# SmoothKen/knn-svc

Measured on AMD Instinct MI355X. Metric: audio-sec converted/sec (xRT) end-to-end, cold target pool, higher is better.
Workload: dtype f32; 1 GPU; north-star point per rank: 30 s source vs 10 min target pool (20 x 30 s), ckpt_type=mix, post_opt_0.2, cold (pool encoded inside the step); seeded random weights of WavLM-Large (6 layers executed) and the 22.9 M-param generator; nq=1500, np_per_rank=30000, wavlm_batch_chunks=32, pipeline_depth=2

## Files before the change

knn_svc_amd/csrc/conv_gemm.hip:

```cpp
#include "gemm_core.h"
#include "gemm3_core.h"
#include "gemm2_core.h"

namespace {

thread_local const char* g_last_epilogue = "";
thread_local const char* g_last_kernel = "";

struct ConvArgs {
    const float* x; long x_bstride, x_gstride; int ldx, t_in, cin, taps, stride, dil, pad; float a_slope;
    const float* w; long w_gstride; int n;
    const float* bias; long bias_gstride; int bias_period;
    float* out; long o_bstride, o_gstride; int ldo, m;
    int act; float act_slope;
    const float* resid; long r_bstride, r_gstride; int ldr;
    int accumulate; float div;
    int groups;
    int convt_u, convt_cout, convt_pad, t_out;
    int K;
    const unsigned short* w3;
    const unsigned short* w2;
    int x_split;
    int out_split;
    int split_from;
// ... 693 lines not shown
#pragma unroll
        for (int it = 0; it < TRIPS; ++it) {
            f32x4 v = *(const lds_f4*)(patch + (it * RSTEP + row_in_trip) * PITCH + c) + bias4;
            if (RES) v += rv[it];
            const int m = mrow0 + it * RSTEP;
            bool ok = nv;
            int off;
            if (CONVT) {
                const int o = m * a.convt_u + phase - a.convt_pad;
                ok = ok && m < a.m && o >= 0 && o < a.t_out;
                off = (o * a.ldo + col) * 4;
            } else off = (m * a.ldo + n) * 4;
            if (a.out_absmax && (!CONVT || ok)) {
#pragma unroll
                for (int e = 0; e < 4; ++e) { const unsigned ab = abs_bits(v[e]); amax = ab > amax ? ab : amax; }
            }
            __builtin_amdgcn_raw_buffer_store_b128(__builtin_bit_cast(u32x4, v), o_rsrc, ok ? off : OOB, 0, 0);
        }
    }
    if (a.out_absmax) publish_absmax(a.out_absmax, amax);
}

template <class G>
__device__ __forceinline__ void conv_gemm2win_body(ConvArgs& a, float* lds) {
    resolve_scales(a);
    const int z = blockIdx.z;
    const int nbz = (int)gridDim.z / a.groups;
    const int g = z / nbz, b = z - g * nbz;
    int m0, n0;
    if (!patch_order_decode<G::BM, G::BN>(a.plain, a.m, a.n, m0, n0)) return;
    const float* xz = a.x + b * a.x_bstride + g * a.x_gstride;
    const unsigned short* wz = a.w2 + (long)g * a.n * (a.K / 32) * 64;

    typename G::acc_t acc[G::TM][G::TN];
    KN_ZERO_ACC(acc, G::TM, G::TN, G::NR)
    Split2BLoader<G::B_P, G::B_PIECES> bl(a.n, a.K, n0, threadIdx.x);
    const int tid = threadIdx.x;
    const int w_off0 = ((m0 - a.pad + (tid >> 3)) * a.ldx + (tid & 7) * 4) * 4;
    if constexpr (G::DEEP)
        G::mainloop_deep(lds, a.cin / 32, a.taps, a.dil, w_off0, a.ldx * 4, bl, acc, FastALoader<1>::desc(a, xz),
                         Split2BLoader<G::B_P, G::B_PIECES>::desc(wz, a.n, a.K), a.a_scale, a.a_slope);
    else
        G::mainloop(lds, a.cin / 32, a.taps, a.dil, w_off0, a.ldx * 4, bl, acc, FastALoader<1>::desc(a, xz),
                    Split2BLoader<G::B_P, G::B_PIECES>::desc(wz, a.n, a.K), a.a_scale, a.a_slope);
    if (a.wide) {
        __syncthreads();
        if (a.resid) conv_epilogue_wide32<G, true>(a, acc, lds, m0, n0, b, g);
        else conv_epilogue_wide32<G, false>(a, acc, lds, m0, n0, b, g);
    } else conv_epilogue_any<G>(a, acc, m0, n0, b, g);
}

template <class G, int MINB>
__global__ __launch_bounds__(256, MINB) void conv_gemm2win_kernel(ConvArgs a) {
    extern __shared__ __attribute__((aligned(16))) float lds[];
    conv_gemm2win_body<G>(a, lds);
}

constexpr int KN_MAX_MULTI = 4;
struct ConvArgsN { ConvArgs b[KN_MAX_MULTI]; };
template <class G, int MINB>
__global__ __launch_bounds__(256, MINB) void conv_gemm2win_multi_kernel(ConvArgsN args) {
    extern __shared__ __attribute__((aligned(16))) float lds[];
    ConvArgs a = args.b[blockIdx.y];
    conv_gemm2win_body<G>(a, lds);
}

template <class G, int MINB>
int launch2win(const ConvArgs* args, int count, int batches, hipStream_t st) {
    const ConvArgs& a = args[0];
    const long gx = cdiv64(a.m, G::BM), gy = cdiv64(a.n, G::BN);
    ConvArgsN ap;
    for (int i = 0; i < KN_MAX_MULTI; ++i) { ap.b[i] = args[i < count ? i : 0]; ap.b[i].plain = patch_order_plain(gx, gy); }
    dim3 grid((unsigned)patch_order_ids(gx, gy), (unsigned)count, (unsigned)(batches * a.groups));
    if (count == 1) {
        if (const int rc = kn_lds_optin<conv_gemm2win_kernel<G, MINB>>(G::LDS_BYTES, "conv_gemm")) return rc;
        hipLaunchKernelGGL((conv_gemm2win_kernel<G, MINB>), grid, dim3(256), G::LDS_BYTES, st, ap.b[0]);
        return knnsvc_check_launch("conv_gemm2win");
    }
    if (const int rc = kn_lds_optin<conv_gemm2win_multi_kernel<G, MINB>>(G::LDS_BYTES, "conv_gemm_multi")) return rc;
    hipLaunchKernelGGL((conv_gemm2win_multi_kernel<G, MINB>), grid, dim3(256), G::LDS_BYTES, st, ap);
    return knnsvc_check_launch("conv_gemm2win_multi");
}

template <class G, int EPI = 0>
__global__ __launch_bounds__(256, 1) void conv_gemm2quad_kernel(ConvArgs a) {
    extern __shared__ __attribute__((aligned(16))) float lds[];
#ifdef KN_QUAD_PROF
    if (threadIdx.x == 0 && blockIdx.x < 8192) kn_quad_prof_buf[blockIdx.x * 4 + 0] = (long long)__builtin_amdgcn_s_memrealtime();
#endif
    resolve_scales(a);
    const int z = blockIdx.z;
    const int b = z / a.groups, g = z - b * a.groups;
    int mt, nt;
    if (!quad_order_decode((int)blockIdx.x, (a.m + G::BM - 1) / G::BM, (a.n + G::BN - 1) / G::BN, mt, nt, (int)blockIdx.z)) return;
    const int m0 = mt * G::BM, n0 = nt * G::BN;
    const float* xz = a.x + b * a.x_bstride + g * a.x_gstride;
    const unsigned short* wz = a.w2 + (long)g * a.n * (a.K / 32) * 64;

    typename G::acc_t acc[G::TM][G::TN];
    KN_ZERO_ACC(acc, G::TM, G::TN, G::NR)
    const int M = a.m, row_step = a.stride * a.ldx * 4, row_pad = a.pad * a.ldx * 4;
    auto row_off = [&](int m) -> int { return m < M ? m * row_step - row_pad : G::OOB_OFF; };
    int c_in_tap = 0, uoff = 0;
    const int cin = a.cin, step_tap = (a.dil * a.ldx - a.cin) * 4;
    auto step = [&](int kt) -> int {
        if (kt > 0) { c_in_tap += 32; uoff += 128; if (c_in_tap == cin) { c_in_tap = 0; uoff += step_tap; } }
        return uoff;
    };
    G::mainloop(lds, a.K / 32, row_off, step, FastALoader<1>::desc(a, xz), uniform_rsrc(wz, (int)((long)a.n * (a.K / 32) * 128)),
                a.n, a.K, m0, n0, acc);
#ifdef KN_T_NOEPI
    { float sink = 0.f;
#pragma unroll
      for (int i = 0; i < G::TM; ++i)
#pragma unroll
          for (int j = 0; j < G::TN; ++j)
#pragma unroll
              for (int r = 0; r < G::NR; ++r) sink += acc[i][j][r];
      if (sink == 123456.789f) a.out[threadIdx.x] = sink; }
#else
    __syncthreads();
#ifdef KN_QUAD_PROF
    if (threadIdx.x == 0 && blockIdx.x < 8192) kn_quad_prof_buf[blockIdx.x * 4 + 2] = (long long)__builtin_amdgcn_s_memrealtime();
#endif
    if constexpr (EPI == 1) conv_epilogue_wide_fast<G, 0, false>(a, acc, lds, m0, n0, b, g);
    else if constexpr (EPI == 2) conv_epilogue_wide_fast<G, 1, false>(a, acc, lds, m0, n0, b, g);
    else if constexpr (EPI == 3) conv_epilogue_wide_fast<G, 0, true>(a, acc, lds, m0, n0, b, g);
    else conv_epilogue_wide<G>(a, acc, lds, m0, n0, b, g);
#ifdef KN_QUAD_PROF
    __builtin_amdgcn_s_waitcnt(0);
    __syncthreads();
    if (threadIdx.x == 0 && blockIdx.x < 8192) kn_quad_prof_buf[blockIdx.x * 4 + 3] = (long long)__builtin_amdgcn_s_memrealtime();
#endif
#endif
}

template <class G, int EPI = 0>
int launch2quad(const ConvArgs& a, int batches, hipStream_t st) {
    if (const int rc = kn_lds_optin<conv_gemm2quad_kernel<G, EPI>>(G::LDS_BYTES, "conv_gemm")) return rc;
    dim3 grid((unsigned)quad_order_ids(cdiv64(a.m, G::BM), cdiv64(a.n, G::BN)), 1, (unsigned)(batches * a.groups));
    hipLaunchKernelGGL((conv_gemm2quad_kernel<G, EPI>), grid, dim3(256), G::LDS_BYTES, st, a);
    return knnsvc_check_launch("conv_gemm2quad");
}

template <class G, bool A2>
int launch2v(const ConvArgs& a, int batches, hipStream_t st) {
    if (const int rc = kn_lds_optin<conv_gemm2_kernel<G, A2>>(G::LDS_BYTES, "conv_gemm")) return rc;
    const long gx = cdiv64(a.m, G::BM), gy = cdiv64(a.n, G::BN);
    ConvArgs ap = a;
    ap.plain = patch_order_plain(gx, gy);
    dim3 grid((unsigned)patch_order_ids(gx, gy), 1, (unsigned)(batches * a.groups));
    hipLaunchKernelGGL((conv_gemm2_kernel<G, A2>), grid, dim3(256), G::LDS_BYTES, st, ap);
    return knnsvc_check_launch("conv_gemm2");
}
template <class G>
int launch2(const ConvArgs& a, int batches, hipStream_t st) {
    return a.x_split ? launch2v<G, true>(a, batches, st) : launch2v<G, false>(a, batches, st);
}

__global__ void split_weight2_kernel(const float* __restrict__ w, long n, int K, float scale, const float* __restrict__ absmax,
                                     unsigned short* __restrict__ out) {
    const long i = (long)blockIdx.x * blockDim.x + threadIdx.x;
    const long groups_per_row = K / 4;
    if (absmax) scale = kn_pick_scale(kn_slot_max(absmax));
    if (i >= n * groups_per_row) return;
    const long row = i / groups_per_row; const int k = (int)(i - row * groups_per_row) * 4;
    g2_u32x2 hi, lo;
    f16x2_split4(*(const f32x4*)(w + row * K + k), scale, hi, lo);
    unsigned short* o = out + row * (long)(K / 32) * 64 + (k / 32) * 64 + (k % 32);
    *(g2_u32x2*)o = hi;
    *(g2_u32x2*)(o + 32) = lo;
}

template <class G>
int launch3(const ConvArgs& a, int batches, hipStream_t st) {
    if (const int rc = kn_lds_optin<conv_gemm3_kernel<G>>(G::LDS_BYTES, "conv_gemm")) return rc;
    dim3 grid((unsigned)cdiv64(a.m, G::BM), (unsigned)cdiv64(a.n, G::BN), (unsigned)(batches * a.groups));
    hipLaunchKernelGGL((conv_gemm3_kernel<G>), grid, dim3(256), G::LDS_BYTES, st, a);
    return knnsvc_check_launch("conv_gemm3");
}

__global__ void split_weight_kernel(const float* __restrict__ w, long n, int K, unsigned short* __restrict__ out) {
    const long i = (long)blockIdx.x * blockDim.x + threadIdx.x;
    const long groups_per_row = K / 4;
    if (i >= n * groups_per_row) return;
    const long row = i / groups_per_row; const int k = (int)(i - row * groups_per_row) * 4;
    const f32x4 v = *(const f32x4*)(w + row * K + k);
    unsigned short* o = out + row * (long)(K / 32) * 96 + (k / 32) * 96 + (k % 32);
#pragma unroll
    for (int e = 0; e < 4; ++e) {
        const unsigned x = __float_as_uint(v[e]);
        const float r1 = v[e] - __uint_as_float(x & 0xFFFF0000u);
        const unsigned y = __float_as_uint(r1);
        const float r2 = r1 - __uint_as_float(y & 0xFFFF0000u);
        o[e] = (unsigned short)(x >> 16);
        o[32 + e] = (unsigned short)(y >> 16);
        o[64 + e] = (unsigned short)(__float_as_uint(r2) >> 16);
    }
}

template <class G, int VEC>
int launch(const ConvArgs& a, int batches, hipStream_t st) {
    dim3 grid((unsigned)cdiv64(a.m, G::BM), (unsigned)cdiv64(a.n, G::BN), (unsigned)(batches * a.groups));
    hipLaunchKernelGGL((conv_gemm_kernel<G, VEC>), grid, dim3(256), G::LDS_BYTES, st, a);
    return knnsvc_check_launch("conv_gemm");
}

using G128 = GemmTile<128, 128, 2, 2, 2, 2>;
using G64 = GemmTile<128, 64, 4, 1, 1, 2>;
using G32 = GemmTile<128, 32, 4, 1, 1, 1>;
using H128 = Gemm3Tile<128, 128, 2, 2, 2, 2>;
using H64 = Gemm3Tile<256, 64, 4, 1, 2, 2>;
using H32 = Gemm3Tile<256, 32, 4, 1, 2, 1>;
using F128 = Gemm2Tile<128, 128, 2, 2, 2, 2>;
using F64S = Gemm2Tile<64, 64, 2, 2, 1, 1>;
using F64 = Gemm2Tile<256, 64, 4, 1, 2, 2>;
using F32 = Gemm2Tile<256, 32, 4, 1, 2, 1>;
using Q256S = Gemm2QuadS;
using W128 = Gemm2Win<128, 128, 2, 2, 2, 2, 64>;
using W160 = Gemm2Win<160, 128, 1, 4, 5, 1, 64>;
using W128S = Gemm2Win<64, 128, 2, 2, 1, 2, 64>;
using W128D = Gemm2Win<64, 128, 2, 2, 1, 2, 64, 1>;
using W64 = Gemm2Win<256, 64, 4, 1, 2, 2, 64>;
using W32 = Gemm2Win<256, 32, 4, 1, 2, 1, 64>;
using W64P = Gemm2Win<256, 64, 4, 1, 2, 2, 128>;

template <class G>
int prepare() {
    int rc = kn_lds_optin<conv_gemm_kernel<G, 8>>(G::LDS_BYTES, "conv_gemm");
    if (!rc) rc = kn_lds_optin<conv_gemm_kernel<G, 4>>(G::LDS_BYTES, "conv_gemm");
    if (!rc) rc = kn_lds_optin<conv_gemm_kernel<G, 1>>(G::LDS_BYTES, "conv_gemm");
    return rc;
}

struct Knobs {
    int quad = 1;
    bool quad_epi = true;
    bool generic_epilogue = false;
    bool win = true;
    bool win_wide = true;
    bool win_small = true, win_deep = true, win160 = true;
    bool gemm_small = true;
    bool loaded = false;
};
Knobs g_knobs;
bool env_off(const char* name) { const char* e = getenv(name); return e && e[0] == '0'; }
void load_knobs() {
    Knobs k;
    const char* q = getenv("KNNSVC_QUAD");
    k.quad = q ? atoi(q) : 1;
    k.quad_epi = !env_off("KNNSVC_QUAD_EPI");
    const char* ep = getenv("KNNSVC_EPILOGUE");
    k.generic_epilogue = ep && ep[0] == 'g';
    k.win = !env_off("KNNSVC_WIN"); k.win_small = !env_off("KNNSVC_WIN_SMALL"); k.win_deep = !env_off("KNNSVC_WIN_DEEP");
    k.win_wide = !env_off("KNNSVC_WIN_WIDE");
    k.win160 = !env_off("KNNSVC_WIN160"); k.gemm_small = !env_off("KNNSVC_GEMM_SMALL");
    k.loaded = true;
    g_knobs = k;
}
const Knobs& knobs() { if (!g_knobs.loaded) load_knobs(); return g_knobs; }

}

extern "C" int knnsvc_reload_knobs(void) { load_knobs(); return KNNSVC_OK; }

static int conv_prep(const knnsvc_conv_desc* d, ConvArgs& a, bool& fast, bool& vec4, bool& quad_ok) {
    KN_REQUIRE(d && d->x && d->w && d->out, "conv_gemm: null operand");
    KN_REQUIRE(d->cin > 0 && d->taps > 0 && d->n > 0 && d->m >= 0 && d->t_in >= 0, "conv_gemm: bad sizes");
    KN_REQUIRE(d->batches > 0 && d->groups > 0, "conv_gemm: batches/groups must be positive");
    KN_REQUIRE((d->ldx >= d->cin || (d->taps == 1 && d->ldx > 0)) && d->stride > 0, "conv_gemm: ldx < cin or stride <= 0");
    KN_REQUIRE((long)d->batches * d->groups <= 65535, "conv_gemm: batches*groups > 65535");
    KN_REQUIRE(cdiv64(d->n, 32) <= 65535, "conv_gemm: n too large for grid.y");
    if (d->convt_u) {
        KN_REQUIRE(d->convt_cout > 0 && d->n % d->convt_cout == 0 && d->n / d->convt_cout == d->convt_u,
                   "conv_gemm: transposed mode needs n == u*cout");
        KN_REQUIRE(d->ldo >= d->convt_cout, "conv_gemm: ldo < cout");
    } else {
        KN_REQUIRE(d->ldo >= d->n, "conv_gemm: ldo < n");
    }
    if (d->resid) KN_REQUIRE(d->ldr > 0, "conv_gemm: resid without ldr");

    a.x = d->x; a.x_bstride = d->x_bstride; a.x_gstride = d->x_gstride; a.ldx = d->ldx; a.t_in = d->t_in;
    a.cin = d->cin; a.taps = d->taps; a.stride = d->stride; a.dil = d->dil; a.pad = d->pad; a.a_slope = d->a_slope;
    a.w = d->w; a.w_gstride = d->w_gstride; a.n = d->n;
    a.bias = d->bias; a.bias_gstride = d->bias_gstride; a.bias_period = d->bias_period;
    a.out = d->out; a.o_bstride = d->o_bstride; a.o_gstride = d->o_gstride; a.ldo = d->ldo; a.m = d->m;
    a.act = d->act; a.act_slope = d->act_slope;
    a.resid = d->resid; a.r_bstride = d->r_bstride; a.r_gstride = d->r_gstride; a.ldr = d->ldr;
    a.accumulate = d->accumulate; a.div = d->div == 0.f ? 1.0f : d->div;
    a.groups = d->groups;
    a.convt_u = d->convt_u; a.convt_cout = d->convt_cout; a.convt_pad = d->convt_pad; a.t_out = d->t_out;
    a.K = d->cin * d->taps;
    a.w3 = (const unsigned short*)d->w_bf16x3;
    a.w2 = (const unsigned short*)d->w_f16x2;
    a.out_scale = 1.0f; a.a_scale = 1.0f; a.w_scale = 1.0f;
    a.x_absmax = nullptr; a.w_absmax = nullptr; a.out_absmax = d->out_absmax; a.x_bound_mul = 1.0f; a.x_bound_add = 0.f;
    a.n_dyn = d->n_dyn; a.dyn_tin_mul = d->dyn_t_in_mul; a.dyn_tin_add = d->dyn_t_in_add; a.dyn_m_mul = d->dyn_m_mul;
    a.dyn_m_add = d->dyn_m_add; a.dyn_tout_mul = d->dyn_t_out_mul;
    if (d->n_dyn) KN_REQUIRE(d->dyn_t_in_mul >= 0 && d->dyn_m_mul >= 0 && d->dyn_t_in_add >= 0 && d->dyn_m_add >= 0 && d->batches == 1,
                             "conv_gemm: dynamic length needs non-negative affine coefficients and batches == 1");
    a.split_scale = d->out_f16x2_scale > 0.f ? d->out_f16x2_scale : KN_F16X2_A_SCALE;
    a.x_split = d->x_f16x2; a.out_split = d->out_f16x2 != 0; a.split_from = d->out_f16x2 > 1 ? d->out_f16x2 : 0;
    KN_REQUIRE(d->out_f16x2 >= 0 && (d->out_f16x2 <= 1 || d->out_f16x2 % 32 == 0), "conv_gemm: out_f16x2 is 0, 1 or the first split column (a multiple of 32)");
    a.wide = 0; a.plain = 0;
    a.lin = !d->convt_u && (long)d->m * d->ldo * 4 < (1L << 31) && (!d->resid || (long)d->m * d->ldr * 4 < (1L << 31)) &&
            !knobs().generic_epilogue;

    vec4 = (d->cin % 4 == 0) && (d->ldx % 4 == 0) && (((uintptr_t)d->x & 15) == 0) &&
                      (((uintptr_t)d->w & 15) == 0) && (d->x_bstride % 4 == 0) && (d->x_gstride % 4 == 0) &&
                      (d->w_gstride % 4 == 0);
    if (const int rc = prepare<G128>()) return rc;
    if (const int rc = prepare<G64>()) return rc;
    if (const int rc = prepare<G32>()) return rc;
    fast = vec4 && (d->cin % 32 == 0) && ((long)d->t_in * d->ldx * 4 < (1L << 30)) &&
                      ((long)d->n * a.K * 4 < (1L << 30)) && ((long)d->m * d->stride * d->ldx * 4 < (1L << 30));
    if (a.out_split)
        KN_REQUIRE(!d->resid && !d->accumulate && a.div == 1.0f && !d->convt_u && d->n % 32 == 0 && d->ldo % 32 == 0 &&
                   ((uintptr_t)d->out & 15) == 0, "conv_gemm: out_f16x2 needs a plain [m, n % 32 == 0] output (no resid/accumulate/div/convt)");
    if (a.out_split) {
        int e2 = 0;
        KN_REQUIRE(frexpf(a.split_scale, &e2) == 0.5f, "conv_gemm: out_f16x2_scale must be a power of two");
        KN_REQUIRE(!a.out_absmax, "conv_gemm: out_absmax is for fp32 outputs (a split output's scale is chosen by the caller)");
    }
    if (a.x_split)
        KN_REQUIRE(fast && a.w2 && d->a_slope == 1.0f,
                   "conv_gemm: x_f16x2 needs the f16x2 fast path (cin % 32 == 0, split weights) and a_slope 1");
    if (fast && a.w2) {
        KN_REQUIRE(d->w_f16x2_scale > 0.f || d->w_absmax, "conv_gemm: w_f16x2 without its scale");
        a.a_scale = d->a_f16x2_scale > 0.f ? d->a_f16x2_scale : KN_F16X2_A_SCALE;
        a.w_scale = d->w_f16x2_scale > 0.f ? d->w_f16x2_scale : 1.0f;
        { int e2 = 0; KN_REQUIRE(frexpf(a.a_scale, &e2) == 0.5f && frexpf(a.w_scale, &e2) == 0.5f, "conv_gemm: f16x2 scales must be powers of two"); }
        a.out_scale = 1.0f / (a.a_scale * a.w_scale);
        a.x_absmax = d->x_absmax; a.w_absmax = d->w_absmax;
        a.x_bound_mul = d->x_bound_mul > 0.f ? d->x_bound_mul : 1.0f; a.x_bound_add = d->x_bound_add;
        KN_REQUIRE(d->x_bound_add >= 0.f && d->x_bound_mul >= 0.f, "conv_gemm: x_bound_mul / x_bound_add must be non-negative");
        quad_ok = a.x_split && a.lin && d->n % 4 == 0 && d->ldo % 4 == 0 && (!d->resid || d->ldr % 4 == 0) && ((uintptr_t)d->out & 15) == 0 &&
            (!d->resid || ((uintptr_t)d->resid & 15) == 0) && d->o_bstride % 4 == 0 && d->o_gstride % 4 == 0 && d->r_bstride % 4 == 0 &&
            d->r_gstride % 4 == 0 && (!a.out_split || a.split_from % 128 == 0) && (!d->bias || d->bias_period || ((uintptr_t)d->bias & 15) == 0) &&
            d->bias_gstride % 4 == 0;
        const bool plain_t = d->convt_u && !d->resid && d->convt_cout % 4 == 0 && (long)d->t_out * d->ldo * 4 < (1L << 31) &&
                             (long)d->m * d->convt_u < (1L << 30);
        a.wide = knobs().win_wide && (a.lin || plain_t) && !a.out_split && d->act == KNNSVC_ACT_NONE && !d->accumulate && a.div == 1.0f &&
            d->n % 4 == 0 && d->ldo % 4 == 0 && ((uintptr_t)d->out & 15) == 0 && d->o_bstride % 4 == 0 && d->o_gstride % 4 == 0 &&
            (!d->resid || (d->ldr % 4 == 0 && ((uintptr_t)d->resid & 15) == 0 && d->r_bstride % 4 == 0 && d->r_gstride % 4 == 0)) &&
            (!d->bias || (d->bias_period % 4 == 0 && ((uintptr_t)d->bias & 15) == 0 && d->bias_gstride % 4 == 0));
        KN_REQUIRE(d->fixed_tile != 2 || quad_ok, "conv_gemm: fixed_tile 2 needs the quad kernel's operand layout (split A, 16-byte rows, n % 4 == 0)");
    }
    return KNNSVC_OK;
}

enum WinShape { WS_NONE, WS_128D, WS_128S, WS_160, WS_128, WS_64, WS_32, WS_64P };
static WinShape win_shape(const knnsvc_conv_desc* d, const ConvArgs& a, long z) {
    if (a.x_split || d->convt_u || d->stride != 1 || d->taps < 3 || d->dil < 1 || d->ldx % 4 != 0 || !knobs().win) return WS_NONE;
    const int halo = (d->taps - 1) * d->dil;
    if (halo <= 64) {
        if (d->n > 64) {
            if (knobs().win_small && cdiv64(d->m, 128) * cdiv64(d->n, 128) * z < 512) {
                if (knobs().win_deep && cdiv64(d->m, 64) * cdiv64(d->n, 128) * z <= 256) return WS_128D;
                return WS_128S;
            }
            const long zz = z * cdiv64(d->n, 128);
            const long r128 = cdiv64(cdiv64(d->m, 128) * zz, 768) * 128, r160 = cdiv64(cdiv64(d->m, 160) * zz, 768) * 160;
            return (knobs().win160 && r160 < r128) ? WS_160 : WS_128;
        }
        return d->n > 32 ? WS_64 : WS_32;
    }
    if (halo <= 128 && d->n > 32 && d->n <= 64) return WS_64P;
    return WS_NONE;
}

static int launch_win(WinShape ws, const ConvArgs* args, int count, int batches, hipStream_t st) {
    const bool x = count > 1;
    switch (ws) {
        case WS_128D: g_last_kernel = x ? "W128Dx" : "W128D"; return launch2win<W128D, 4>(args, count, batches, st);
        case WS_128S: g_last_kernel = x ? "W128Sx" : "W128S"; return launch2win<W128S, 4>(args, count, batches, st);
        case WS_160: g_last_kernel = x ? "W160x" : "W160"; return launch2win<W160, 3>(args, count, batches, st);
        case WS_128: g_last_kernel = x ? "W128x" : "W128"; return launch2win<W128, 3>(args, count, batches, st);
        case WS_64: g_last_kernel = x ? "W64x" : "W64"; return launch2win<W64, 2>(args, count, batches, st);
        case WS_32: g_last_kernel = x ? "W32x" : "W32"; return launch2win<W32, 3>(args, count, batches, st);
        case WS_64P: g_last_kernel = x ? "W64Px" : "W64P"; return launch2win<W64P, 2>(args, count, batches, st);
        case WS_NONE: break;
    }
    return knnsvc_fail(KNNSVC_EINVAL, "conv_gemm: no windowed kernel for this shape");
}

extern "C" int knnsvc_conv_gemm(const knnsvc_conv_desc* d, void* stream) {
    ConvArgs a;
    bool fast = false, vec4 = false, quad_ok = false;
    const int rc = conv_prep(d, a, fast, vec4, quad_ok);
    if (rc) return rc;
    if (d->m == 0) return KNNSVC_OK;
    hipStream_t st = (hipStream_t)stream;
    g_last_epilogue = "";
    if (fast && a.w2) {
        if (d->fixed_tile != 1 && quad_ok) {
            const Knobs& kb = knobs();
            if (d->fixed_tile == 2 || kb.quad == 2 || (kb.quad == 1 && d->n >= 256 && a.K >= 1024)) {
                const bool fast_epi = kb.quad_epi && !d->accumulate && a.div == 1.0f && !a.out_absmax &&
                                      (d->act == KNNSVC_ACT_NONE || d->act == KNNSVC_ACT_GELU) && !(d->resid && d->act != KNNSVC_ACT_NONE);
                g_last_kernel = "Q256S";
                if (fast_epi && d->resid) return launch2quad<Q256S, 3>(a, d->batches, st);
                if (fast_epi && d->act == KNNSVC_ACT_GELU) return launch2quad<Q256S, 2>(a, d->batches, st);
                if (fast_epi) return launch2quad<Q256S, 1>(a, d->batches, st);
                return launch2quad<Q256S>(a, d->batches, st);
            }
        }
        g_last_epilogue = a.wide ? "patch" : "lane";
        const WinShape ws = win_shape(d, a, (long)d->batches * d->groups);
        if (ws != WS_NONE) return launch_win(ws, &a, 1, d->batches, st);
        if (d->n > 64 && cdiv64(d->m, 128) * cdiv64(d->n, 128) * d->batches * d->groups < 256) {
            if (knobs().gemm_small) { g_last_kernel = "F64S"; return launch2<F64S>(a, d->batches, st); }
        }
        g_last_kernel = d->n > 64 ? (a.x_split ? "F128a2" : "F128") : d->n > 32 ? "F64" : "F32";
        if (d->n > 64) return launch2<F128>(a, d->batches, st);
        if (d->n > 32) return launch2<F64>(a, d->batches, st);
        return launch2<F32>(a, d->batches, st);
    }
    if (fast && a.w3) {
        g_last_kernel = d->n > 64 ? "H128" : d->n > 32 ? "H64" : "H32";
        if (d->n > 64) return launch3<H128>(a, d->batches, st);
        if (d->n > 32) return launch3<H64>(a, d->batches, st);
        return launch3<H32>(a, d->batches, st);
    }
    g_last_kernel = d->n > 64 ? (fast ? "G128v8" : vec4 ? "G128v4" : "G128v1") : d->n > 32 ? (fast ? "G64v8" : vec4 ? "G64v4" : "G64v1") : (fast ? "G32v8" : vec4 ? "G32v4" : "G32v1");
    if (d->n > 64) return fast ? launch<G128, 8>(a, d->batches, st) : vec4 ? launch<G128, 4>(a, d->batches, st) : launch<G128, 1>(a, d->batches, st);
    if (d->n > 32) return fast ? launch<G64, 8>(a, d->batches, st) : vec4 ? launch<G64, 4>(a, d->batches, st) : launch<G64, 1>(a, d->batches, st);
    return fast ? launch<G32, 8>(a, d->batches, st) : vec4 ? launch<G32, 4>(a, d->batches, st) : launch<G32, 1>(a, d->batches, st);
}

extern "C" const char* knnsvc_conv_gemm_last_kernel(void) { return g_last_kernel; }
extern "C" const char* knnsvc_conv_gemm_last_epilogue(void) { return g_last_epilogue; }

extern "C" int knnsvc_conv_gemm_multi(const knnsvc_conv_desc* descs, int32_t count, void* stream) {
    KN_REQUIRE(descs && count >= 1 && count <= KN_MAX_MULTI, "conv_gemm_multi: 1..4 descriptors");
    ConvArgsN an;
    bool one_grid = true;
    for (int i = 0; i < count; ++i) {
        bool fast = false, vec4 = false, quad_ok = false;
        const int rc = conv_prep(&descs[i], an.b[i], fast, vec4, quad_ok);
        if (rc) return rc;
        const knnsvc_conv_desc& d = descs[i];
        one_grid = one_grid && fast && an.b[i].w2 && d.batches == 1 && d.groups == 1 && d.m == descs[0].m && d.n == descs[0].n && d.m > 0 &&
                   win_shape(&d, an.b[i], count) != WS_NONE && win_shape(&d, an.b[i], count) == win_shape(&descs[0], an.b[0], count);
    }
    if (!one_grid || count == 1) {
        for (int i = 0; i < count; ++i) { const int rc = knnsvc_conv_gemm(&descs[i], stream); if (rc) return rc; }
        return KNNSVC_OK;
    }
    return launch_win(win_shape(&descs[0], an.b[0], count), an.b, count, 1, (hipStream_t)stream);
}

extern "C" int knnsvc_split_weight_bf16x3(const float* w, int64_t rows, int32_t K, void* out, void* stream) {
    KN_REQUIRE(w && out && rows > 0 && K > 0 && K % 32 == 0, "split_weight: K must be a positive multiple of 32");
    KN_REQUIRE(((uintptr_t)w & 15) == 0, "split_weight: 16-byte alignment");
    const long groups = rows * (K / 4);
    hipLaunchKernelGGL(split_weight_kernel, dim3((unsigned)cdiv64(groups, 256)), dim3(256), 0, (hipStream_t)stream,
                       w, (long)rows, K, (unsigned short*)out);
    return knnsvc_check_launch("split_weight");
}

extern "C" int knnsvc_split_weight_f16x2(const float* w, int64_t rows, int32_t K, float scale, void* out, void* stream) {
    KN_REQUIRE(w && out && rows > 0 && K > 0 && K % 32 == 0, "split_weight: K must be a positive multiple of 32");
    KN_REQUIRE(((uintptr_t)w & 15) == 0 && ((uintptr_t)out & 15) == 0, "split_weight: 16-byte alignment");
    int e = 0;
    KN_REQUIRE(scale > 0.f && frexpf(scale, &e) == 0.5f, "split_weight: scale must be a power of two");
    const long groups = rows * (K / 4);
    hipLaunchKernelGGL(split_weight2_kernel, dim3((unsigned)cdiv64(groups, 256)), dim3(256), 0, (hipStream_t)stream,
                       w, (long)rows, K, scale, (const float*)nullptr, (unsigned short*)out);
    return knnsvc_check_launch("split_weight2");
}

extern "C" int knnsvc_split_f16x2_dyn(const float* w, int64_t rows, int32_t K, const float* absmax, void* out, void* stream) {
    KN_REQUIRE(w && out && absmax && rows > 0 && K > 0 && K % 32 == 0, "split_f16x2_dyn: K must be a positive multiple of 32");
    KN_REQUIRE(((uintptr_t)w & 15) == 0 && ((uintptr_t)out & 15) == 0, "split_f16x2_dyn: 16-byte alignment");
    const long groups = rows * (K / 4);
    hipLaunchKernelGGL(split_weight2_kernel, dim3((unsigned)cdiv64(groups, 256)), dim3(256), 0, (hipStream_t)stream,
                       w, (long)rows, K, 1.0f, absmax, (unsigned short*)out);
    return knnsvc_check_launch("split_f16x2_dyn");
}

namespace {
__global__ __launch_bounds__(256) void absmax_kernel(const float* __restrict__ x, long rows, int cols, int ld, int vec,
                                                     float* __restrict__ slot) {
    const int c4 = vec ? cols >> 2 : 0;
    slot = kn_stripe(slot);
    unsigned m = 0;
    const long n4 = rows * c4;
// ... 271 lines not shown
```

knn_svc_amd/csrc/gemm2_core.h:

```cpp
#pragma once
#include "common.h"

typedef _Float16 f16x8 __attribute__((ext_vector_type(8)));
typedef _Float16 f16x2_t __attribute__((ext_vector_type(2)));
typedef float f32x2_t __attribute__((ext_vector_type(2)));
typedef unsigned g2_u32x4 __attribute__((ext_vector_type(4)));
typedef unsigned g2_u32x2 __attribute__((ext_vector_type(2)));

constexpr float KN_F16X2_A_SCALE = 16.0f;

__device__ __forceinline__ void f16x2_split4(f32x4 v, float scale, g2_u32x2& hi, g2_u32x2& lo) {
    f32x2_t a = {v[0], v[1]}, b = {v[2], v[3]};
    a *= scale; b *= scale;
    const f16x2_t ha = __builtin_convertvector(a, f16x2_t), hb = __builtin_convertvector(b, f16x2_t);
    const f32x2_t ra = a - __builtin_convertvector(ha, f32x2_t), rb = b - __builtin_convertvector(hb, f32x2_t);
    const f16x2_t la = __builtin_convertvector(ra, f16x2_t), lb = __builtin_convertvector(rb, f16x2_t);
    hi = (g2_u32x2){__builtin_bit_cast(unsigned, ha), __builtin_bit_cast(unsigned, hb)};
    lo = (g2_u32x2){__builtin_bit_cast(unsigned, la), __builtin_bit_cast(unsigned, lb)};
}

typedef __attribute__((address_space(3))) char g2_lds_c;
typedef __attribute__((address_space(3))) g2_u32x4 g2_lds_u4;
typedef __attribute__((address_space(3))) g2_u32x2 g2_lds_u2;

// ... 84 lines not shown
template <int BM_, int BN_, int WM_, int WN_, int TM_, int TN_>
struct Gemm2Tile : Acc32<WN_, TM_, TN_> {
    typedef f32x16 acc_t;
    static constexpr int NR = 16;
    static constexpr int BM = BM_, BN = BN_, WM = WM_, WN = WN_, TM = TM_, TN = TN_;
    static constexpr int BK = 32, PITCH = 144, THREADS = 256;
    static_assert(WM * WN == 4 && WM * TM * 32 == BM && WN * TN * 32 == BN, "tile shape");
    static constexpr int A_F4 = BM / 32;
    static constexpr int B_PIECES = BN * 8;
    static constexpr int B_P = (B_PIECES + 255) / 256;
    static constexpr int LDS_BYTES = (BM + BN) * PITCH;

    __device__ __forceinline__ static void split_store(g2_lds_c* dst, f32x4 v, float a_scale) {
        g2_u32x2 hi, lo;
        f16x2_split4(v, a_scale, hi, lo);
        *(g2_lds_u2*)(dst) = hi;
        *(g2_lds_u2*)(dst + 64) = lo;
    }

    template <bool A2 = false, class ALoad, class BLoad, class RA, class RB>
    __device__ __forceinline__ static void mainloop(float* lds_generic, int nk, ALoad& aload, BLoad& bload,
                                                    f32x16 (&acc)[TM][TN], RA ra_desc, RB rb_desc, float a_scale) {
        g2_lds_c* lds = (g2_lds_c*)lds_generic;
        const int tid = threadIdx.x;
        const int a_st = (tid >> 3) * PITCH + (tid & 7) * (A2 ? 16 : 8);
        const int lane = tid & 63, wave = tid >> 6;
        const int wm = wave / WN, wn = wave % WN;
        const int li = lane & 31, lh = lane >> 5;
        const int a_frag = (wm * TM * 32 + li) * PITCH + lh * 16;
        const int b_frag = BM * PITCH + (wn * TN * 32 + li) * PITCH + lh * 16;

        f32x4 ra[A_F4];
        g2_u32x4 rb[B_P];
#define KN_STAGE2()                                                                                               \
    {                                                                                                            \
        _Pragma("unroll") for (int j = 0; j < A_F4; ++j) {                                                       \
            if constexpr (A2) *(g2_lds_u4*)(lds + a_st + 32 * j * PITCH) = __builtin_bit_cast(g2_u32x4, ra[j]);   \
            else split_store(lds + a_st + 32 * j * PITCH, aload.finish(ra[j]), a_scale);                         \
        }                                                                                                        \
        KN_SPLIT_B_STAGE(rb, BM * PITCH)                                                                         \
    }
        aload.begin(0); bload.begin(0);
#pragma unroll
        for (int j = 0; j < A_F4; ++j) ra[j] = aload(0, j, ra_desc);
#pragma unroll
        for (int j = 0; j < B_P; ++j) rb[j] = bload(0, j, rb_desc);
        KN_STAGE2();
        __syncthreads();

        for (int kt = 0; kt < nk; ++kt) {
            const bool more = (kt + 1 < nk);
            if (more) {
                aload.begin(kt + 1); bload.begin(kt + 1);
#pragma unroll
                for (int j = 0; j < A_F4; ++j) ra[j] = aload(kt + 1, j, ra_desc);
#pragma unroll
                for (int j = 0; j < B_P; ++j) rb[j] = bload(kt + 1, j, rb_desc);
            }
            KN_F16X2_SLAB_MMA(lds + a_frag, lds + b_frag)
            __syncthreads();
            if (more) KN_STAGE2();
            __syncthreads();
        }
#undef KN_STAGE2
    }
};

struct Gemm2QuadS {
    typedef f32x4 acc_t;
    static constexpr int NR = 4;
    static constexpr int BM = 256, BN = 256, WM = 2, WN = 2, TM = 8, TN = 8;
    static constexpr int EPI_TN = 4;
    static constexpr int ROW = 128, NW = 4, THREADS = 256;
    static constexpr int A_P = BM * ROW / 1024 / NW, B_P = BN * ROW / 1024 / NW;
    static_assert(A_P == 8 && B_P == 8, "schedule below is written for 8 + 8 pieces");
    static constexpr int BOFF = BM * ROW;
    static constexpr int STAGE = (BM + BN) * ROW;
    static constexpr int EPI_BYTES = NW * 32 * (EPI_TN * 32 + 4) * 4;
    static constexpr int LDS_BYTES = 2 * STAGE > EPI_BYTES ? 2 * STAGE : EPI_BYTES;
    static constexpr int OOB_OFF = 0x40000000;

    typedef __attribute__((address_space(3))) char lds_c;
    typedef __attribute__((address_space(3))) g2_u32x4 lds_u4;

    template <class RowOff, class Step, class RA, class RB>
    __device__ __forceinline__ static void mainloop(float* lds_generic, int nk, RowOff a_row_off, Step a_step, RA ra_desc,
                                                    RB rb_desc, int N, int K, int m0, int n0, f32x4 (&acc)[TM][TN]) {
        lds_c* lds = (lds_c*)lds_generic;
        const int tid = threadIdx.x, lane = tid & 63, wave = __builtin_amdgcn_readfirstlane(tid >> 6);
        const int wm = wave / WN, wn = wave % WN;
        const int a_row = (wm * 128 + (lane & 15)) * ROW;
        const int b_row = BOFF + (wn * 128 + (lane & 15)) * ROW;
        int x_off[2];
#pragma unroll
        for (int p = 0; p < 2; ++p) x_off[p] = ((p * 4 + (lane >> 4)) ^ (lane & 7)) * 16;
        int a_src[A_P], b_src[B_P];
        const int row_bytes = (K / 32) * 128;
#pragma unroll
        for (int t = 0; t < A_P; ++t) {
            const int row = (wave * A_P + t) * 8 + (lane >> 3);
            const int ro = a_row_off(m0 + row);
            a_src[t] = ro == OOB_OFF ? OOB_OFF : ro + (lane & 7) * 16;
        }
#pragma unroll
        for (int t = 0; t < B_P; ++t) {
            const int row = (wave * B_P + t) * 8 + (lane >> 3);
            b_src[t] = (n0 + row < N) ? (n0 + row) * row_bytes + (lane & 7) * 16 : OOB_OFF;
        }
        const int st_dst = wave * 8 * 1024 + (lane >> 3) * ROW + (((lane & 7) ^ (lane >> 3)) * 16);
        int ua = 0;
        int a_issued = 0, b_issued = 0;
        g2_u32x4 st[8];
#define KN_S_LOAD_A(T) { st[T] = __builtin_amdgcn_raw_buffer_load_b128(ra_desc, a_src[T] + ua, 0, 0); }
#define KN_S_LOAD_B(T) { st[T] = __builtin_amdgcn_raw_buffer_load_b128(rb_desc, b_src[T], b_issued * 128, 0); }
#define KN_S_WRITE(T, OFF) { *(lds_u4*)(lds + (OFF) + st_dst + (T) * 1024) = st[T]; }
        f16x8 fa[2][4][2], fb[2][4][2];
#define KN_S_READ_A(SET, STG, II, I) { _Pragma("unroll") for (int p = 0; p < 2; ++p) fa[SET][I][p] = __builtin_bit_cast(f16x8, *(const lds_u4*)(lds + (STG) + a_row + ((II) * 4 + (I)) * 16 * ROW + x_off[p])); }
#define KN_S_READ_B(SET, STG, JJ, J) { _Pragma("unroll") for (int p = 0; p < 2; ++p) fb[SET][J][p] = __builtin_bit_cast(f16x8, *(const lds_u4*)(lds + (STG) + b_row + ((JJ) * 4 + (J)) * 16 * ROW + x_off[p])); }
#define KN_S_MFMA1(C, A, B) asm volatile("v_mfma_f32_16x16x32_f16 %0, %1, %2, %0" : "+a"(C) : "v"(A), "v"(B));
#define KN_S_MFMA(AS, BS, I, J)                                                                                           \
    {                                                                                                                     \
        KN_S_MFMA1(acc[(AS) * 4 + (I)][(BS) * 4 + (J)], fa[AS][I][1], fb[BS][J][0])                 \
        KN_S_MFMA1(acc[(AS) * 4 + (I)][(BS) * 4 + (J)], fa[AS][I][0], fb[BS][J][1])                                       \
        KN_S_MFMA1(acc[(AS) * 4 + (I)][(BS) * 4 + (J)], fa[AS][I][0], fb[BS][J][0])                                       \
    }
        ua = a_step(0);
#pragma unroll
        for (int t = 0; t < 8; ++t) KN_S_LOAD_A(t)
        a_issued = 1;
#pragma unroll
        for (int t = 0; t < 8; ++t) KN_S_WRITE(t, 0)
#pragma unroll
        for (int t = 0; t < 8; ++t) KN_S_LOAD_B(t)
        b_issued = 1;
#pragma unroll
        for (int t = 0; t < 8; ++t) KN_S_WRITE(t, BOFF)
        if (nk > 1) {
            ua = a_step(1);
#pragma unroll
            for (int t = 0; t < 8; ++t) KN_S_LOAD_A(t)
            a_issued = 2;
        }
        __builtin_amdgcn_s_waitcnt(0xC07F);
        __builtin_amdgcn_s_barrier();
#ifdef KN_QUAD_PROF
        if (threadIdx.x == 0 && blockIdx.x < 8192) kn_quad_prof_buf[blockIdx.x * 4 + 1] = (long long)__builtin_amdgcn_s_memrealtime();
#endif
#pragma unroll
        for (int i = 0; i < 4; ++i) KN_S_READ_A(0, 0, 0, i)
#pragma unroll
        for (int j = 0; j < 4; ++j) KN_S_READ_B(0, 0, 0, j)

#define KN_S_SLAB(FB, HN, ML)                                                                                             \
    {                                                                                                                     \
        constexpr int cstg = (FB) * STAGE, nstg = (1 - (FB)) * STAGE;              \
                                                                                                     \
        _Pragma("unroll") for (int t = 0; t < 16; ++t) {                                                                  \
            KN_S_MFMA(0, FB, t >> 2, t & 3)                                                                               \
            __builtin_amdgcn_sched_barrier(0);                                                                            \
            if (t < 8) { if (t < 4) KN_S_READ_B(1 - (FB), cstg, 1 - (FB), t) }                                            \
            else if (HN) KN_S_WRITE(t - 8, nstg)                                                                          \
            __builtin_amdgcn_sched_barrier(0);                                                                            \
        }                                                                                                                 \
                                                                                                   \
        _Pragma("unroll") for (int t = 0; t < 16; ++t) {                                                                  \
            KN_S_MFMA(0, 1 - (FB), t >> 2, t & 3)                                                                         \
            __builtin_amdgcn_sched_barrier(0);                                                                            \
            if (t < 8) { if (HN) KN_S_LOAD_B(t) }                                                                         \
            else if (t < 12) KN_S_READ_A(1, cstg, 1, t - 8)                                                               \
            __builtin_amdgcn_sched_barrier(0);                                                                            \
        }                                                                                                                 \
        if (HN) ++b_issued;                                                                                               \
        if (ML) ua = a_step(a_issued);                                                                                    \
                                                                                                   \
        _Pragma("unroll") for (int t = 0; t < 16; ++t) {                                                                  \
            KN_S_MFMA(1, 1 - (FB), t >> 2, t & 3)                                                                         \
            __builtin_amdgcn_sched_barrier(0);                                                                            \
            if (t >= 8) {                                                                                                 \
                if (HN) KN_S_WRITE(t - 8, nstg + BOFF)                                                                    \
                if (ML) KN_S_LOAD_A(t - 8)                                                                                \
            }                                                                                                             \
            __builtin_amdgcn_sched_barrier(0);                                                                            \
        }                                                                                                                 \
        if (ML) ++a_issued;                                                                                               \
        if (HN) { __builtin_amdgcn_s_waitcnt(0xC07F); __builtin_amdgcn_s_barrier(); }                                     \
                     \
        _Pragma("unroll") for (int t = 0; t < 16; ++t) {                                                                  \
            KN_S_MFMA(1, FB, t >> 2, t & 3)                                                                               \
            __builtin_amdgcn_sched_barrier(0);                                                                            \
            if (HN) {                                                                                                     \
                if (t < 4) KN_S_READ_A(0, nstg, 0, t)                                                                     \
                else if (t >= 8 && t < 12) KN_S_READ_B(1 - (FB), nstg, 1 - (FB), t - 8)                                   \
            }                                                                                                             \
            __builtin_amdgcn_sched_barrier(0);                                                                            \
        }                                                                                                                 \
    }
        int s = 0;
        for (; s + 1 < nk; s += 2) {
            KN_S_SLAB(0, true, true)
            KN_S_SLAB(1, true, true)
        }
        if (s < nk) KN_S_SLAB(0, true, true)
#undef KN_S_SLAB
#undef KN_S_MFMA
#undef KN_S_MFMA1
#undef KN_S_READ_A
#undef KN_S_READ_B
#undef KN_S_WRITE
#undef KN_S_LOAD_A
#undef KN_S_LOAD_B
    }

    __device__ __forceinline__ static int acc_row(int wave, int lane, int i, int r) { return (wave / WN) * 128 + i * 16 + 4 * (lane >> 4) + r; }
    __device__ __forceinline__ static int acc_col(int wave, int lane, int j) { return (wave % WN) * 128 + j * 16 + (lane & 15); }

};

template <int BM_, int BN_, int WM_, int WN_, int TM_, int TN_, int HALO_, int DEEP_ = 0>
struct Gemm2Win : Acc32<WN_, TM_, TN_> {
    static constexpr int DEEP = DEEP_;
    typedef f32x16 acc_t;
    static constexpr int NR = 16;
    static constexpr int BM = BM_, BN = BN_, WM = WM_, WN = WN_, TM = TM_, TN = TN_, HALO = HALO_;
    static constexpr int BK = 32, PITCH = 144, THREADS = 256;
    static_assert(WM * WN == 4 && WM * TM * 32 == BM && WN * TN * 32 == BN && HALO % 32 == 0, "tile shape");
    static constexpr int WR = BM + HALO;
    static constexpr int W_F4 = WR / 32;
    static constexpr int B_PIECES = BN * 8;
    static constexpr int B_P = (B_PIECES + 255) / 256;
    static constexpr int BOFF = WR * PITCH;
    static constexpr int LDS_BYTES = (WR + BN) * PITCH;

#define KN_WIN_LOAD(CS)                                                                                        \
    _Pragma("unroll") for (int j = 0; j < W_F4; ++j)                                                          \
        rw[j] = __builtin_bit_cast(f32x4, __builtin_amdgcn_raw_buffer_load_b128(ra_desc, w_off0 + j * 32 * row_bytes + (CS) * 128, 0, 0));
#define KN_WIN_STAGE()                                                                                         \
    _Pragma("unroll") for (int j = 0; j < W_F4; ++j) {                                                        \
        f32x4 v = rw[j];                                                                                      \
        if (a_slope != 1.0f) { _Pragma("unroll") for (int e = 0; e < 4; ++e) v[e] = v[e] > 0.f ? v[e] : v[e] * a_slope; } \
        g2_u32x2 hi, lo;                                                                                      \
        f16x2_split4(v, a_scale, hi, lo);                                                                     \
        *(g2_lds_u2*)(lds + w_st + 32 * j * PITCH) = hi;                                                      \
        *(g2_lds_u2*)(lds + w_st + 32 * j * PITCH + 64) = lo;                                                 \
    }

    template <class BLoad, class RA, class RB>
    __device__ __forceinline__ static void mainloop(float* lds_generic, int ncs, int taps, int dil, int w_off0, int row_bytes,
                                                    BLoad& bload, f32x16 (&acc)[TM][TN], RA ra_desc, RB rb_desc,
                                                    float a_scale, float a_slope) {
        g2_lds_c* lds = (g2_lds_c*)lds_generic;
        const int tid = threadIdx.x;
        const int w_st = (tid >> 3) * PITCH + (tid & 7) * 8;
        const int lane = tid & 63, wave = tid >> 6;
        const int wm = wave / WN, wn = wave % WN;
        const int li = lane & 31, lh = lane >> 5;
        const int a_frag = (wm * TM * 32 + li) * PITCH + lh * 16;
        const int b_frag = BOFF + (wn * TN * 32 + li) * PITCH + lh * 16;
        const int tap_step = dil * PITCH;

        f32x4 rw[W_F4];
        g2_u32x4 rb[B_P];
        KN_WIN_LOAD(0)
        KN_SPLIT_B_LOAD(rb, 0)
        KN_WIN_STAGE()
        KN_SPLIT_B_STAGE(rb, BOFF)
        __syncthreads();
        for (int cs = 0; cs < ncs; ++cs) {
            const bool more_cs = cs + 1 < ncs;
            if (more_cs) { KN_WIN_LOAD(cs + 1) }
            int tap_off = 0;
            for (int tap = 0; tap < taps; ++tap, tap_off += tap_step) {
                const bool last_tap = tap + 1 == taps;
                const bool more = !last_tap || more_cs;
#ifndef KN_WIN_NOBLOAD
                if (more) {
                    const int slab = last_tap ? (cs + 1) : ((tap + 1) * ncs + cs);
                    KN_SPLIT_B_LOAD(rb, slab)
                }
#endif
                KN_F16X2_SLAB_MMA(lds + a_frag + tap_off, lds + b_frag)
#ifndef KN_WIN_NOBAR
                __syncthreads();
#endif
#ifndef KN_WIN_NOBLOAD
                if (more) { KN_SPLIT_B_STAGE(rb, BOFF) }
#endif
                if (last_tap && more_cs) { KN_WIN_STAGE() }
#ifndef KN_WIN_NOBAR
                __syncthreads();
#endif
            }
// ... 87 lines not shown
```

Measured before the change: 925.7 x real-time.

## Load A tiles directly into LDS via buffer_load_lds in quad conv GEMM

Adds an A_DMA path to the Q256S quad conv-GEMM mainloop. It uses raw buffer loads that write straight into LDS, with an XOR-swizzled source offset, instead of loading into registers and then storing to LDS. The direct loads are issued during the second MFMA half of each slab, and the waitcnt is changed to wait on vmcnt. The aim is to cut VGPR pressure and the ds_write instructions for the A operand. The risks are stage hazards, since the DMA targets the current stage, and a changed synchronisation pattern; the path is on by default and can be turned off with KNNSVC_QUAD_ADMA=0.

```diff
diff --git a/knn_svc_amd/csrc/conv_gemm.hip b/knn_svc_amd/csrc/conv_gemm.hip
--- a/knn_svc_amd/csrc/conv_gemm.hip
+++ b/knn_svc_amd/csrc/conv_gemm.hip
@@ -799,7 +799,7 @@
     return knnsvc_check_launch("conv_gemm2win_multi");
 }
 
-template <class G, int EPI = 0>
+template <class G, int EPI = 0, bool ADMA = false>
 __global__ __launch_bounds__(256, 1) void conv_gemm2quad_kernel(ConvArgs a) {
     extern __shared__ __attribute__((aligned(16))) float lds[];
 #ifdef KN_QUAD_PROF
@@ -824,8 +824,8 @@
         if (kt > 0) { c_in_tap += 32; uoff += 128; if (c_in_tap == cin) { c_in_tap = 0; uoff += step_tap; } }
         return uoff;
     };
-    G::mainloop(lds, a.K / 32, row_off, step, FastALoader<1>::desc(a, xz), uniform_rsrc(wz, (int)((long)a.n * (a.K / 32) * 128)),
-                a.n, a.K, m0, n0, acc);
+    G::template mainloop<ADMA>(lds, a.K / 32, row_off, step, FastALoader<1>::desc(a, xz), uniform_rsrc(wz, (int)((long)a.n * (a.K / 32) * 128)),
+                               a.n, a.K, m0, n0, acc);
 #ifdef KN_T_NOEPI
     { float sink = 0.f;
 #pragma unroll
@@ -852,12 +852,16 @@
 #endif
 }
 
+template <class G, int EPI, bool ADMA>
+int launch2quad_as(const ConvArgs& a, int batches, hipStream_t st) {
+    if (const int rc = kn_lds_optin<conv_gemm2quad_kernel<G, EPI, ADMA>>(G::LDS_BYTES, "conv_gemm")) return rc;
+    dim3 grid((unsigned)quad_order_ids(cdiv64(a.m, G::BM), cdiv64(a.n, G::BN)), 1, (unsigned)(batches * a.groups));
+    hipLaunchKernelGGL((conv_gemm2quad_kernel<G, EPI, ADMA>), grid, dim3(256), G::LDS_BYTES, st, a);
+    return knnsvc_check_launch("conv_gemm2quad");
+}
 template <class G, int EPI = 0>
-int launch2quad(const ConvArgs& a, int batches, hipStream_t st) {
-    if (const int rc = kn_lds_optin<conv_gemm2quad_kernel<G, EPI>>(G::LDS_BYTES, "conv_gemm")) return rc;
-    dim3 grid((unsigned)quad_order_ids(cdiv64(a.m, G::BM), cdiv64(a.n, G::BN)), 1, (unsigned)(batches * a.groups));
-    hipLaunchKernelGGL((conv_gemm2quad_kernel<G, EPI>), grid, dim3(256), G::LDS_BYTES, st, a);
-    return knnsvc_check_launch("conv_gemm2quad");
+int launch2quad(const ConvArgs& a, int batches, hipStream_t st, bool a_dma) {
+    return a_dma ? launch2quad_as<G, EPI, true>(a, batches, st) : launch2quad_as<G, EPI, false>(a, batches, st);
 }
 
 template <class G, bool A2>
@@ -958,6 +962,7 @@
     bool win_wide = true;
     bool win_small = true, win_deep = true, win160 = true;
     bool gemm_small = true;
+    int quad_adma = -1;
     bool loaded = false;
 };
 Knobs g_knobs;
@@ -972,6 +977,8 @@
     k.win = !env_off("KNNSVC_WIN"); k.win_small = !env_off("KNNSVC_WIN_SMALL"); k.win_deep = !env_off("KNNSVC_WIN_DEEP");
     k.win_wide = !env_off("KNNSVC_WIN_WIDE");
     k.win160 = !env_off("KNNSVC_WIN160"); k.gemm_small = !env_off("KNNSVC_GEMM_SMALL");
+    const char* ad = getenv("KNNSVC_QUAD_ADMA");
+    k.quad_adma = (ad && (ad[0] == '0' || ad[0] == '1')) ? ad[0] - '0' : -1;
     k.loaded = true;
     g_knobs = k;
 }
@@ -1086,6 +1093,8 @@
     return WS_NONE;
 }
 
+static bool quad_a_dma() { return knobs().quad_adma != 0; }
+
 static int launch_win(WinShape ws, const ConvArgs* args, int count, int batches, hipStream_t st) {
     const bool x = count > 1;
     switch (ws) {
@@ -1116,10 +1125,11 @@
                 const bool fast_epi = kb.quad_epi && !d->accumulate && a.div == 1.0f && !a.out_absmax &&
                                       (d->act == KNNSVC_ACT_NONE || d->act == KNNSVC_ACT_GELU) && !(d->resid && d->act != KNNSVC_ACT_NONE);
                 g_last_kernel = "Q256S";
-                if (fast_epi && d->resid) return launch2quad<Q256S, 3>(a, d->batches, st);
-                if (fast_epi && d->act == KNNSVC_ACT_GELU) return launch2quad<Q256S, 2>(a, d->batches, st);
-                if (fast_epi) return launch2quad<Q256S, 1>(a, d->batches, st);
-                return launch2quad<Q256S>(a, d->batches, st);
+                const bool a_dma = quad_a_dma();
+                if (fast_epi && d->resid) return launch2quad<Q256S, 3>(a, d->batches, st, a_dma);
+                if (fast_epi && d->act == KNNSVC_ACT_GELU) return launch2quad<Q256S, 2>(a, d->batches, st, a_dma);
+                if (fast_epi) return launch2quad<Q256S, 1>(a, d->batches, st, a_dma);
+                return launch2quad<Q256S>(a, d->batches, st, a_dma);
             }
         }
         g_last_epilogue = a.wide ? "patch" : "lane";
diff --git a/knn_svc_amd/csrc/gemm2_core.h b/knn_svc_amd/csrc/gemm2_core.h
--- a/knn_svc_amd/csrc/gemm2_core.h
+++ b/knn_svc_amd/csrc/gemm2_core.h
@@ -190,8 +190,9 @@
 
     typedef __attribute__((address_space(3))) char lds_c;
     typedef __attribute__((address_space(3))) g2_u32x4 lds_u4;
-
-    template <class RowOff, class Step, class RA, class RB>
+    typedef __attribute__((address_space(3))) void lds_dma;
+
+    template <bool A_DMA = false, class RowOff, class Step, class RA, class RB>
     __device__ __forceinline__ static void mainloop(float* lds_generic, int nk, RowOff a_row_off, Step a_step, RA ra_desc,
                                                     RB rb_desc, int N, int K, int m0, int n0, f32x4 (&acc)[TM][TN]) {
         lds_c* lds = (lds_c*)lds_generic;
@@ -203,12 +204,14 @@
 #pragma unroll
         for (int p = 0; p < 2; ++p) x_off[p] = ((p * 4 + (lane >> 4)) ^ (lane & 7)) * 16;
         int a_src[A_P], b_src[B_P];
+        int a_dma[A_DMA ? A_P : 1];
         const int row_bytes = (K / 32) * 128;
 #pragma unroll
         for (int t = 0; t < A_P; ++t) {
             const int row = (wave * A_P + t) * 8 + (lane >> 3);
             const int ro = a_row_off(m0 + row);
             a_src[t] = ro == OOB_OFF ? OOB_OFF : ro + (lane & 7) * 16;
+            if constexpr (A_DMA) a_dma[t] = ro == OOB_OFF ? OOB_OFF : ro + (((lane & 7) ^ (lane >> 3)) * 16);
         }
 #pragma unroll
         for (int t = 0; t < B_P; ++t) {
@@ -222,6 +225,7 @@
 #define KN_S_LOAD_A(T) { st[T] = __builtin_amdgcn_raw_buffer_load_b128(ra_desc, a_src[T] + ua, 0, 0); }
 #define KN_S_LOAD_B(T) { st[T] = __builtin_amdgcn_raw_buffer_load_b128(rb_desc, b_src[T], b_issued * 128, 0); }
 #define KN_S_WRITE(T, OFF) { *(lds_u4*)(lds + (OFF) + st_dst + (T) * 1024) = st[T]; }
+#define KN_S_DMA_A(T, STG) { __builtin_amdgcn_raw_ptr_buffer_load_lds(ra_desc, (lds_dma*)(lds + (STG) + wave * (A_P * 1024) + (T) * 1024), 16, a_dma[T] + ua, 0, 0, 0); }
         f16x8 fa[2][4][2], fb[2][4][2];
 #define KN_S_READ_A(SET, STG, II, I) { _Pragma("unroll") for (int p = 0; p < 2; ++p) fa[SET][I][p] = __builtin_bit_cast(f16x8, *(const lds_u4*)(lds + (STG) + a_row + ((II) * 4 + (I)) * 16 * ROW + x_off[p])); }
 #define KN_S_READ_B(SET, STG, JJ, J) { _Pragma("unroll") for (int p = 0; p < 2; ++p) fb[SET][J][p] = __builtin_bit_cast(f16x8, *(const lds_u4*)(lds + (STG) + b_row + ((JJ) * 4 + (J)) * 16 * ROW + x_off[p])); }
@@ -246,7 +250,7 @@
         if (nk > 1) {
             ua = a_step(1);
 #pragma unroll
-            for (int t = 0; t < 8; ++t) KN_S_LOAD_A(t)
+            for (int t = 0; t < 8; ++t) { if constexpr (A_DMA) KN_S_DMA_A(t, STAGE) else KN_S_LOAD_A(t) }
             a_issued = 2;
         }
         __builtin_amdgcn_s_waitcnt(0xC07F);
@@ -267,7 +271,7 @@
             KN_S_MFMA(0, FB, t >> 2, t & 3)                                                                               \
             __builtin_amdgcn_sched_barrier(0);                                                                            \
             if (t < 8) { if (t < 4) KN_S_READ_B(1 - (FB), cstg, 1 - (FB), t) }                                            \
-            else if (HN) KN_S_WRITE(t - 8, nstg)                                                                          \
+            else if (HN && !A_DMA) KN_S_WRITE(t - 8, nstg)                                                                \
             __builtin_amdgcn_sched_barrier(0);                                                                            \
         }                                                                                                                 \
                                                                                                    \
@@ -286,12 +290,13 @@
             __builtin_amdgcn_sched_barrier(0);                                                                            \
             if (t >= 8) {                                                                                                 \
                 if (HN) KN_S_WRITE(t - 8, nstg + BOFF)                                                                    \
-                if (ML) KN_S_LOAD_A(t - 8)                                                                                \
+                if (ML && !A_DMA) KN_S_LOAD_A(t - 8)                                                                      \
             }                                                                                                             \
             __builtin_amdgcn_sched_barrier(0);                                                                            \
         }                                                                                                                 \
         if (ML) ++a_issued;                                                                                               \
-        if (HN) { __builtin_amdgcn_s_waitcnt(0xC07F); __builtin_amdgcn_s_barrier(); }                                     \
+            \
+        if (HN) { __builtin_amdgcn_s_waitcnt(A_DMA ? 0x0070 : 0xC07F); __builtin_amdgcn_s_barrier(); }                    \
                      \
         _Pragma("unroll") for (int t = 0; t < 16; ++t) {                                                                  \
             KN_S_MFMA(1, FB, t >> 2, t & 3)                                                                               \
@@ -300,6 +305,8 @@
                 if (t < 4) KN_S_READ_A(0, nstg, 0, t)                                                                     \
                 else if (t >= 8 && t < 12) KN_S_READ_B(1 - (FB), nstg, 1 - (FB), t - 8)                                   \
             }                                                                                                             \
+             \
+            if (A_DMA && (ML) && (t & 4)) KN_S_DMA_A((t >> 3) * 4 + (t & 3), cstg)                                        \
             __builtin_amdgcn_sched_barrier(0);                                                                            \
         }                                                                                                                 \
     }
@@ -309,12 +316,14 @@
             KN_S_SLAB(1, true, true)
         }
         if (s < nk) KN_S_SLAB(0, true, true)
+        if constexpr (A_DMA) __builtin_amdgcn_s_waitcnt(0x0070);
 #undef KN_S_SLAB
 #undef KN_S_MFMA
 #undef KN_S_MFMA1
 #undef KN_S_READ_A
 #undef KN_S_READ_B
 #undef KN_S_WRITE
+#undef KN_S_DMA_A
 #undef KN_S_LOAD_A
 #undef KN_S_LOAD_B
     }
```

Result: no change. 934.7 x real-time (median of 6 runs) (+1.0%).
